# swapUniba/Deep_CBRS_Amar_Renaissance

Hardware: AMD Instinct MI355X
Metric: (user,item) pairs scored/sec, ML-1M basic-gnn 2-layer, 1/2/4/8 MI355X (higher is better)
Workload: dtype f32; 1 GPU; ml1m(s=64) user-item graph: N=590592 nodes, nnz(A_hat)=55909934, 12089292 test pairs; econfigs/basic-gnn.yaml grid1 BasicGCN d=8 L=2 concat, dense [24,24], clf [48,48]; one propagation + per-entity towers + all pairs (shuffled order) per step (hoisted); scale=64, parallelism=single GPU (step replayed from a hipGraph)

## Files before the change

deep_cbrs_amar_renaissance_amd/csrc/amar_chain.hip:

```cpp
#include "amar_common.h"
#include <stdlib.h>
#include <string.h>

namespace {

typedef float f32x4 __attribute__((ext_vector_type(4)));

constexpr int CHAIN_MAX_LAYERS = 8;
constexpr int CHAIN_MAX_SEG = 8;

struct ChainArgs {
    const float *A; int64_t lda; int Da; const int32_t *ids_a; int base_a;
    int n_seg; const float *seg[CHAIN_MAX_SEG]; int64_t seg_ld[CHAIN_MAX_SEG]; int seg_off[CHAIN_MAX_SEG + 1];
    const float *B; int64_t ldb; int Db; const int32_t *ids_b; int base_b;
    const float *wpack; int wpack_floats;
    int sum_inputs, in_act;
    int n_layers;
    int kt[CHAIN_MAX_LAYERS], nt[CHAIN_MAX_LAYERS], act[CHAIN_MAX_LAYERS];
    int w_off[CHAIN_MAX_LAYERS], b_off[CHAIN_MAX_LAYERS];
    int has_dot, dot_off, dot_bias_off, dot_act, dot_kt;
    int n_out;
    float *out; int64_t ldo; int64_t P;
    const int32_t *out_index;
};
// ... 132 lines not shown

__device__ __forceinline__ float relu_bits(float v) { return __int_as_float(max(__float_as_int(v), 0)); }

constexpr int chain_shape(int nl, int t0, int t1, int t2 = 0, int t3 = 0) { return nl | t0 << 3 | t1 << 6 | t2 << 9 | t3 << 12; }
constexpr int shape_nl(int s) { return s & 7; }
constexpr int shape_t(int s, int j) { return (s >> (3 * (j + 1))) & 7; }
constexpr int shape_maxt(int s) {
    int m = 0;
    for (int j = 0; j <= shape_nl(s); ++j) m = shape_t(s, j) > m ? shape_t(s, j) : m;
    return m;
}

template <int SHAPE, int PT, bool LASTLIN, bool SEG>
__global__ __launch_bounds__(256) void chain_rows_kernel(const ChainArgs a) {
    constexpr int NL = shape_nl(SHAPE), T0 = shape_t(SHAPE, 0), TN = shape_t(SHAPE, NL), MAXT = shape_maxt(SHAPE);
    extern __shared__ __attribute__((aligned(16))) float w_lds[];
    for (int i = threadIdx.x * 4; i < a.wpack_floats; i += blockDim.x * 4)
        *reinterpret_cast<float4 *>(&w_lds[i]) = *reinterpret_cast<const float4 *>(a.wpack + i);
    __syncthreads();

    const int lane = threadIdx.x & 63, g = lane >> 4, col = lane & 15;
    constexpr uint32_t rows_per_wave = 16 * PT;
    const uint32_t stride = gridDim.x * 4 * rows_per_wave;
    const uint32_t P = (uint32_t)a.P, last = P - 1;
    const uint32_t lda = (uint32_t)a.lda * 4u;
    const int f_last = 16 * (T0 - 1) + 4 * g;
    const bool tail_ok = f_last < a.Da;
    const char *Ag = reinterpret_cast<const char *>(a.A) + 16 * g;
    const int tail_off = tail_ok ? 64 * (T0 - 1) : -16 * g;
    const char *seg_base[SEG ? T0 : 1];
    uint32_t seg_ldb[SEG ? T0 : 1];
    if constexpr (SEG) {
#pragma unroll
        for (int t = 0; t < T0; ++t) {
            const int f = 16 * t + 4 * g;
            int sidx = 0;
            for (int j = 1; j < a.n_seg; ++j) sidx = (f < a.Da && f >= a.seg_off[j]) ? j : sidx;
            seg_base[t] = reinterpret_cast<const char *>(a.seg[sidx] + (f < a.Da ? f - a.seg_off[sidx] : 0));
            seg_ldb[t] = (uint32_t)a.seg_ld[sidx] * 4u;
        }
    }

    f32x4 xin[MAXT][PT];
    auto gather = [&](uint32_t b) {
#pragma unroll
        for (int pt = 0; pt < PT; ++pt) {
            const uint32_t p = min(b + 16 * pt + col, last);
            const uint32_t row = a.ids_a ? (uint32_t)(a.ids_a[p] - a.base_a) : p;
            const char *pa = Ag + (uint64_t)row * lda;
#pragma unroll
            for (int t = 0; t < T0; ++t) {
                if constexpr (SEG) xin[t][pt] = *reinterpret_cast<const f32x4 *>(seg_base[t] + (uint64_t)row * seg_ldb[t]);
                else xin[t][pt] = *reinterpret_cast<const f32x4 *>(pa + (t == T0 - 1 ? tail_off : 64 * t));
            }
        }
    };

    uint32_t base = (blockIdx.x * 4 + (threadIdx.x >> 6)) * rows_per_wave;
    if (base >= P) return;
    gather(base);
    for (; base < P; base += stride) {
        f32x4 x[MAXT][PT];
#pragma unroll
        for (int l = 0; l < NL; ++l) {
            const int KT = shape_t(SHAPE, l), NT = shape_t(SHAPE, l + 1);
            const float *wl = w_lds + a.w_off[l];
            const float *bl = w_lds + a.b_off[l];
            f32x4 y[MAXT][PT];
#pragma unroll
            for (int m = 0; m < MAXT; ++m) {
                if (m < NT) {
                    const f32x4 b4 = *reinterpret_cast<const f32x4 *>(bl + 16 * m + 4 * g);
#pragma unroll
                    for (int pt = 0; pt < PT; ++pt) y[m][pt] = b4;
#pragma unroll
                    for (int t = 0; t < MAXT; ++t) {
                        if (t < KT) {
                            const f32x4 w4 = *reinterpret_cast<const f32x4 *>(wl + ((m * KT + t) * 64 + lane) * 4);
#pragma unroll
                            for (int r = 0; r < 4; ++r)
#pragma unroll
                                for (int pt = 0; pt < PT; ++pt) {
                                    float xv = l == 0 ? xin[t][pt][r] : x[t][pt][r];
                                    if (l == 0 && t == T0 - 1) xv = tail_ok ? xv : 0.f;
                                    y[m][pt] = __builtin_amdgcn_mfma_f32_16x16x4f32(w4[r], xv, y[m][pt], 0, 0, 0);
                                }
                        }
                    }
                }
            }
            if (l == 0) gather(base + stride);
#pragma unroll
            for (int m = 0; m < MAXT; ++m)
#pragma unroll
                for (int pt = 0; pt < PT; ++pt)
                    if (m < NT) {
#pragma unroll
                        for (int r = 0; r < 4; ++r) x[m][pt][r] = (LASTLIN && l == NL - 1) ? y[m][pt][r] : relu_bits(y[m][pt][r]);
                    }
        }
#pragma unroll
        for (int pt = 0; pt < PT; ++pt) {
            const uint32_t p = base + 16 * pt + col;
            float *po = a.out + (int64_t)p * a.ldo + 4 * g;
#pragma unroll
            for (int m = 0; m < TN; ++m)
                if (p < P && 16 * m + 4 * g < a.n_out) *reinterpret_cast<f32x4 *>(po + 16 * m) = x[m][pt];
        }
    }
}


typedef uint32_t u32x4 __attribute__((ext_vector_type(4)));
typedef __bf16 bf16x8 __attribute__((ext_vector_type(8)));

struct Split3 { uint32_t h, m, l; };
typedef float f32x2 __attribute__((ext_vector_type(2)));
typedef uint32_t u32x2 __attribute__((ext_vector_type(2)));
__device__ __forceinline__ Split3 split_pair(float a, float b) {
    const f32x2 x = {a, b};
    const u32x2 xb = __builtin_bit_cast(u32x2, x);
    Split3 q;
    q.h = __builtin_amdgcn_perm(xb[1], xb[0], 0x07060302u);
    const f32x2 r1 = x - __builtin_bit_cast(f32x2, xb & 0xffff0000u);
    const u32x2 r1b = __builtin_bit_cast(u32x2, r1);
    q.m = __builtin_amdgcn_perm(r1b[1], r1b[0], 0x07060302u);
    const f32x2 r2 = r1 - __builtin_bit_cast(f32x2, r1b & 0xffff0000u);
    const u32x2 r2b = __builtin_bit_cast(u32x2, r2);
    q.l = __builtin_amdgcn_perm(r2b[1], r2b[0], 0x07060302u);
    return q;
}

struct Split3x4 { u32x4 h, m, l; };
__device__ __forceinline__ Split3x4 split_tiles(const f32x4 &t0, const f32x4 &t1) {
    const Split3 q0 = split_pair(t0[0], t0[1]), q1 = split_pair(t0[2], t0[3]), q2 = split_pair(t1[0], t1[1]), q3 = split_pair(t1[2], t1[3]);
    Split3x4 o;
    o.h[0] = q0.h; o.h[1] = q1.h; o.h[2] = q2.h; o.h[3] = q3.h;
    o.m[0] = q0.m; o.m[1] = q1.m; o.m[2] = q2.m; o.m[3] = q3.m;
    o.l[0] = q0.l; o.l[1] = q1.l; o.l[2] = q2.l; o.l[3] = q3.l;
    return o;
}
__device__ __forceinline__ f32x4 split_mfma(const u32x4 *w, const Split3x4 &x, f32x4 acc) {
    const bf16x8 wh = __builtin_bit_cast(bf16x8, w[0]), wm = __builtin_bit_cast(bf16x8, w[64]), wl = __builtin_bit_cast(bf16x8, w[128]);
    const bf16x8 xh = __builtin_bit_cast(bf16x8, x.h), xm = __builtin_bit_cast(bf16x8, x.m), xl = __builtin_bit_cast(bf16x8, x.l);
    acc = __builtin_amdgcn_mfma_f32_16x16x32_bf16(wl, xh, acc, 0, 0, 0);
    acc = __builtin_amdgcn_mfma_f32_16x16x32_bf16(wh, xl, acc, 0, 0, 0);
    acc = __builtin_amdgcn_mfma_f32_16x16x32_bf16(wm, xm, acc, 0, 0, 0);
    acc = __builtin_amdgcn_mfma_f32_16x16x32_bf16(wm, xh, acc, 0, 0, 0);
    acc = __builtin_amdgcn_mfma_f32_16x16x32_bf16(wh, xm, acc, 0, 0, 0);
    acc = __builtin_amdgcn_mfma_f32_16x16x32_bf16(wh, xh, acc, 0, 0, 0);
    return acc;
}

template <int MAXT, int PT, bool SCATTER, bool SPLIT>
__global__ __launch_bounds__(256) void chain_pipe_kernel(const ChainArgs a) {
    extern __shared__ __attribute__((aligned(16))) float w_lds[];
    for (int i = threadIdx.x * 4; i < a.wpack_floats; i += blockDim.x * 4)
        *reinterpret_cast<float4 *>(&w_lds[i]) = *reinterpret_cast<const float4 *>(a.wpack + i);
    __syncthreads();

    const int lane = threadIdx.x & 63, g = lane >> 4, col = lane & 15;
    constexpr int KS = (MAXT + 1) / 2;
    constexpr bool BIASK = SPLIT && (MAXT & 1);
    u32x4 *frag = reinterpret_cast<u32x4 *>(w_lds + ((a.wpack_floats + 3) & ~3));
    if (SPLIT) {
        for (int idx = threadIdx.x >> 6; idx < a.n_layers * MAXT * KS; idx += 4) {
            const int l = idx / (MAXT * KS), m = (idx % (MAXT * KS)) / KS, sk = idx % KS;
            const float *wl = w_lds + a.w_off[l];
            const f32x4 wa = *reinterpret_cast<const f32x4 *>(wl + ((m * MAXT + 2 * sk) * 64 + lane) * 4);
            f32x4 wb = {0.f, 0.f, 0.f, 0.f};
            if (2 * sk + 1 < MAXT) wb = *reinterpret_cast<const f32x4 *>(wl + ((m * MAXT + 2 * sk + 1) * 64 + lane) * 4);
            else if (BIASK && g == 0) wb[0] = w_lds[a.b_off[l] + 16 * m + col];
            u32x4 *dst = frag + idx * 3 * 64 + lane;
            const Split3 q0 = split_pair(wa[0], wa[1]), q1 = split_pair(wa[2], wa[3]), q2 = split_pair(wb[0], wb[1]), q3 = split_pair(wb[2], wb[3]);
            u32x4 h, mm, lo;
            h[0] = q0.h; h[1] = q1.h; h[2] = q2.h; h[3] = q3.h;
            mm[0] = q0.m; mm[1] = q1.m; mm[2] = q2.m; mm[3] = q3.m;
            lo[0] = q0.l; lo[1] = q1.l; lo[2] = q2.l; lo[3] = q3.l;
            dst[0] = h; dst[64] = mm; dst[128] = lo;
        }
        __syncthreads();
    }
    constexpr uint32_t pairs_per_wave = 16 * PT;
    const uint32_t wave0 = blockIdx.x * 4 + (threadIdx.x >> 6);
    const uint32_t stride = gridDim.x * 4 * pairs_per_wave;
    const uint32_t P = (uint32_t)a.P, last = P - 1;
    const char *Ag = reinterpret_cast<const char *>(a.A + 4 * g), *Bg = reinterpret_cast<const char *>(a.B + 4 * g);
    const uint32_t lda = (uint32_t)a.lda * 4u, ldb = (uint32_t)a.ldb * 4u;
    const char *ids_a = reinterpret_cast<const char *>(a.ids_a), *ids_b = reinterpret_cast<const char *>(a.ids_b);

    auto load_ids = [&](uint32_t b, int32_t (&ra)[PT], int32_t (&rb)[PT]) {
#pragma unroll
        for (int pt = 0; pt < PT; ++pt) {
            const uint32_t off = min(b + 16 * pt + col, last) << 2;
            ra[pt] = *reinterpret_cast<const int32_t *>(ids_a + off);
            rb[pt] = *reinterpret_cast<const int32_t *>(ids_b + off);
        }
    };
    auto issue = [&](const int32_t (&ra)[PT], const int32_t (&rb)[PT], f32x4 (&va)[MAXT][PT], f32x4 (&vb)[MAXT][PT]) {
#pragma unroll
        for (int pt = 0; pt < PT; ++pt) {
            const char *pa = Ag + (uint64_t)(uint32_t)(ra[pt] - a.base_a) * lda;
            const char *pb = Bg + (uint64_t)(uint32_t)(rb[pt] - a.base_b) * ldb;
#pragma unroll
            for (int t = 0; t < MAXT; ++t) {
                va[t][pt] = *reinterpret_cast<const f32x4 *>(pa + 64 * t);
                vb[t][pt] = *reinterpret_cast<const f32x4 *>(pb + 64 * t);
            }
        }
    };
#define AMAR_SPLIT_MFMA(W, X)                                                                                                   \
    _Pragma("unroll") for (int pt = 0; pt < PT; ++pt)                                                                           \
        y[m][pt] = __builtin_amdgcn_mfma_f32_16x16x32_bf16(W, __builtin_bit_cast(bf16x8, X[pt]), y[m][pt], 0, 0, 0)
    auto step = [&](uint32_t base, int32_t (&ra)[PT], int32_t (&rb)[PT], f32x4 (&va)[MAXT][PT], f32x4 (&vb)[MAXT][PT],
                    f32x4 (&na)[MAXT][PT], f32x4 (&nb)[MAXT][PT]) {
        int32_t out_row = 0;
        if (SCATTER) out_row = *reinterpret_cast<const int32_t *>(reinterpret_cast<const char *>(a.out_index) +
                                                                  (min(base + 16 * min(g, PT - 1) + col, last) << 2));
        f32x4 x[MAXT][PT];
#pragma unroll
        for (int t = 0; t < MAXT; ++t)
#pragma unroll
            for (int pt = 0; pt < PT; ++pt) {
                f32x4 v = va[t][pt] + vb[t][pt];
#pragma unroll
                for (int r = 0; r < 4; ++r) v[r] = relu_bits(v[r]);
                x[t][pt] = v;
            }
        issue(ra, rb, na, nb);
        load_ids(base + 2 * stride, ra, rb);
        for (int l = 0; SPLIT && l < a.n_layers; ++l) {
            u32x4 xq[3][KS][PT];
#pragma unroll
            for (int sk = 0; sk < KS; ++sk)
#pragma unroll
                for (int pt = 0; pt < PT; ++pt) {
#pragma unroll
                    for (int hf = 0; hf < 2; ++hf) {
                        const int t = 2 * sk + hf;
                        if (t < MAXT) {
                            const Split3 q0 = split_pair(x[t][pt][0], x[t][pt][1]), q1 = split_pair(x[t][pt][2], x[t][pt][3]);
                            xq[0][sk][pt][2 * hf] = q0.h; xq[1][sk][pt][2 * hf] = q0.m; xq[2][sk][pt][2 * hf] = q0.l;
                            xq[0][sk][pt][2 * hf + 1] = q1.h; xq[1][sk][pt][2 * hf + 1] = q1.m; xq[2][sk][pt][2 * hf + 1] = q1.l;
                        } else {
                            xq[0][sk][pt][2] = (BIASK && g == 0) ? 0x00003f80u : 0u;
                            xq[0][sk][pt][3] = 0u;
                            xq[1][sk][pt][2] = xq[1][sk][pt][3] = xq[2][sk][pt][2] = xq[2][sk][pt][3] = 0u;
                        }
                    }
                }
            const u32x4 *fl = frag + (size_t)l * MAXT * KS * 3 * 64 + lane;
            const float *bl = w_lds + a.b_off[l];
            f32x4 y[MAXT][PT];
#pragma unroll
            for (int m = 0; m < MAXT; ++m) {
                f32x4 b4 = {0.f, 0.f, 0.f, 0.f};
                if (!BIASK) b4 = *reinterpret_cast<const f32x4 *>(bl + 16 * m + 4 * g);
#pragma unroll
                for (int pt = 0; pt < PT; ++pt) y[m][pt] = b4;
#pragma unroll
                for (int sk = 0; sk < KS; ++sk) {
                    const bf16x8 wh = __builtin_bit_cast(bf16x8, fl[((m * KS + sk) * 3 + 0) * 64]);
                    const bf16x8 wm = __builtin_bit_cast(bf16x8, fl[((m * KS + sk) * 3 + 1) * 64]);
                    const bf16x8 wo = __builtin_bit_cast(bf16x8, fl[((m * KS + sk) * 3 + 2) * 64]);
                    AMAR_SPLIT_MFMA(wo, xq[0][sk]);
                    AMAR_SPLIT_MFMA(wh, xq[2][sk]);
                    AMAR_SPLIT_MFMA(wm, xq[1][sk]);
                    AMAR_SPLIT_MFMA(wm, xq[0][sk]);
                    AMAR_SPLIT_MFMA(wh, xq[1][sk]);
                    AMAR_SPLIT_MFMA(wh, xq[0][sk]);
                }
            }
#pragma unroll
            for (int m = 0; m < MAXT; ++m)
#pragma unroll
                for (int pt = 0; pt < PT; ++pt)
#pragma unroll
                    for (int r = 0; r < 4; ++r) x[m][pt][r] = relu_bits(y[m][pt][r]);
        }
        for (int l = 0; !SPLIT && l < a.n_layers; ++l) {
            const float *wl = w_lds + a.w_off[l] + lane * 4;
            const float *bl = w_lds + a.b_off[l];
            f32x4 y[MAXT][PT];
            f32x4 wnext = *reinterpret_cast<const f32x4 *>(wl);
#pragma unroll
            for (int m = 0; m < MAXT; ++m) {
                const f32x4 b4 = *reinterpret_cast<const f32x4 *>(bl + 16 * m + 4 * g);
#pragma unroll
                for (int pt = 0; pt < PT; ++pt) y[m][pt] = b4;
#pragma unroll
                for (int t = 0; t < MAXT; ++t) {
                    const f32x4 w4 = wnext;
                    if (m * MAXT + t + 1 < MAXT * MAXT) {
                        wnext = *reinterpret_cast<const f32x4 *>(wl + (m * MAXT + t + 1) * 256);
                        __builtin_amdgcn_sched_barrier(0);
                    }
#pragma unroll
                    for (int r = 0; r < 4; ++r)
#pragma unroll
                        for (int pt = 0; pt < PT; ++pt)
                            y[m][pt] = __builtin_amdgcn_mfma_f32_16x16x4f32(w4[r], x[t][pt][r], y[m][pt], 0, 0, 0);
                }
            }
#pragma unroll
            for (int m = 0; m < MAXT; ++m)
#pragma unroll
                for (int pt = 0; pt < PT; ++pt)
#pragma unroll
                    for (int r = 0; r < 4; ++r) x[m][pt][r] = relu_bits(y[m][pt][r]);
        }
        if (a.has_dot) {
            const float *wd = w_lds + a.dot_off;
            const float bd = w_lds[a.dot_bias_off];
            f32x4 w4[MAXT];
#pragma unroll
            for (int t = 0; t < MAXT; ++t) w4[t] = *reinterpret_cast<const f32x4 *>(wd + 16 * t + 4 * g);
            float s[PT];
#pragma unroll
            for (int pt = 0; pt < PT; ++pt) {
                float acc = 0.f;
#pragma unroll
                for (int t = 0; t < MAXT; ++t)
#pragma unroll
                    for (int r = 0; r < 4; ++r) acc = fmaf(x[t][pt][r], w4[t][r], acc);
                acc += __shfl_xor(acc, 16, 64);
                acc += __shfl_xor(acc, 32, 64);
                s[pt] = acc;
            }
            float z = s[0];
#pragma unroll
            for (int pt = 1; pt < PT; ++pt) z = g == pt ? s[pt] : z;
            z += bd;
            z = chain_act(z, a.dot_act);
            const uint32_t p = base + 16 * g + col;
            if (g < PT && p < P) a.out[(SCATTER ? (int64_t)out_row : (int64_t)p) * a.ldo] = z;
        } else {
#pragma unroll
            for (int pt = 0; pt < PT; ++pt) {
                const uint32_t p = base + 16 * pt + col;
#pragma unroll
                for (int m = 0; m < MAXT; ++m) {
                    const int f = 16 * m + 4 * g;
                    if (p < P && f < a.n_out) *reinterpret_cast<f32x4 *>(a.out + chain_out_row(a, p) * a.ldo + f) = x[m][pt];
                }
            }
        }
    };
#undef AMAR_SPLIT_MFMA

    uint32_t base = wave0 * pairs_per_wave;
    if (base >= P) return;
    f32x4 va[MAXT][PT], vb[MAXT][PT];
    int32_t ra[PT], rb[PT];
    load_ids(base, ra, rb);
    issue(ra, rb, va, vb);
    load_ids(base + stride, ra, rb);
    for (; base < P; base += stride) step(base, ra, rb, va, vb, va, vb);
}

struct DualArgs {
    const float *A[2]; int64_t lda[2]; const int32_t *ida[2]; int base_a[2];
    const float *B[2]; int64_t ldb[2]; const int32_t *idb[2]; int base_b[2];
    int D, tb, in_act;
    int n_branch; int bw_off[2][CHAIN_MAX_LAYERS], bb_off[2][CHAIN_MAX_LAYERS], b_act[CHAIN_MAX_LAYERS];
    int n_trunk, tt; int tw_off[CHAIN_MAX_LAYERS], tbias_off[CHAIN_MAX_LAYERS], t_act[CHAIN_MAX_LAYERS];
    int dot_off, dot_bias_off, dot_act;
    const float *wpack; int wpack_floats;
    float *out; int64_t ldo; int64_t P;
    const int32_t *out_index;
    int n_frag, tail_floats;
    int bw_frag[2][CHAIN_MAX_LAYERS], bb_tail[2][CHAIN_MAX_LAYERS], tw_frag[CHAIN_MAX_LAYERS], tb_tail[CHAIN_MAX_LAYERS], dot_tail, dot_bias_tail;
};

template <int PT>
__global__ __launch_bounds__(1024) void dual_chain_kernel(const DualArgs a) {
    constexpr int T = 4;
    extern __shared__ __attribute__((aligned(16))) float w_lds[];
    for (int i = threadIdx.x * 4; i < a.wpack_floats; i += blockDim.x * 4)
        *reinterpret_cast<float4 *>(&w_lds[i]) = *reinterpret_cast<const float4 *>(a.wpack + i);
    __syncthreads();
    const int lane = threadIdx.x & 63, g = lane >> 4, col = lane & 15;
    const int64_t pairs_per_wave = 16 * PT;
    const int wpb = blockDim.x >> 6;
    const int64_t wave0 = (int64_t)blockIdx.x * wpb + (threadIdx.x >> 6);
    const int64_t stride = (int64_t)gridDim.x * wpb * pairs_per_wave;
    const int TB = a.tb, TT = a.tt;

    for (int64_t base = wave0 * pairs_per_wave; base < a.P; base += stride) {
        f32x4 xb[2][T][PT];
#pragma unroll
        for (int br = 0; br < 2; ++br) {
#pragma unroll
            for (int pt = 0; pt < PT; ++pt) {
                const int64_t p = base + 16 * pt + col;
                const bool ok = p < a.P;
                const int64_t ra = ok ? (a.ida[br] ? (int64_t)a.ida[br][p] - a.base_a[br] : p) : 0;
                const int64_t rb = ok ? (a.idb[br] ? (int64_t)a.idb[br][p] - a.base_b[br] : p) : 0;
#pragma unroll
                for (int t = 0; t < T; ++t) {
                    const int f = 16 * t + 4 * g;
                    f32x4 v = {0.f, 0.f, 0.f, 0.f};
                    if (t < TB && ok && f < a.D) {
                        const f32x4 va = *reinterpret_cast<const f32x4 *>(a.A[br] + ra * a.lda[br] + f);
                        const f32x4 vb = *reinterpret_cast<const f32x4 *>(a.B[br] + rb * a.ldb[br] + f);
                        v = va + vb;
#pragma unroll
                        for (int r = 0; r < 4; ++r) v[r] = chain_act(v[r], a.in_act);
                    }
                    xb[br][t][pt] = v;
                }
            }
            for (int l = 0; l < a.n_branch; ++l) {
                const float *wl = w_lds + a.bw_off[br][l], *bl = w_lds + a.bb_off[br][l];
                f32x4 y[T][PT];
#pragma unroll
                for (int m = 0; m < T; ++m) {
                    if (m < TB) {
                        const f32x4 b4 = *reinterpret_cast<const f32x4 *>(bl + 16 * m + 4 * g);
#pragma unroll
                        for (int pt = 0; pt < PT; ++pt) y[m][pt] = b4;
#pragma unroll
                        for (int t = 0; t < T; ++t)
                            if (t < TB) {
                                const f32x4 w4 = *reinterpret_cast<const f32x4 *>(wl + ((m * TB + t) * 64 + lane) * 4);
#pragma unroll
                                for (int r = 0; r < 4; ++r)
#pragma unroll
                                    for (int pt = 0; pt < PT; ++pt)
                                        y[m][pt] = __builtin_amdgcn_mfma_f32_16x16x4f32(w4[r], xb[br][t][pt][r], y[m][pt], 0, 0, 0);
                            }
                    }
                }
#pragma unroll
                for (int m = 0; m < T; ++m)
#pragma unroll
                    for (int pt = 0; pt < PT; ++pt) {
                        f32x4 v = {0.f, 0.f, 0.f, 0.f};
                        if (m < TB) {
                            v = y[m][pt];
#pragma unroll
                            for (int r = 0; r < 4; ++r) v[r] = chain_act(v[r], a.b_act[l]);
                        }
                        xb[br][m][pt] = v;
                    }
            }
        }
        f32x4 x[T][PT];
        for (int l = 0; l < a.n_trunk; ++l) {
            const float *wl = w_lds + a.tw_off[l], *bl = w_lds + a.tbias_off[l];
            const int KT = l == 0 ? 2 * TB : TT;
            f32x4 y[T][PT];
#pragma unroll
            for (int m = 0; m < T; ++m) {
                if (m < TT) {
                    const f32x4 b4 = *reinterpret_cast<const f32x4 *>(bl + 16 * m + 4 * g);
#pragma unroll
                    for (int pt = 0; pt < PT; ++pt) y[m][pt] = b4;
#pragma unroll
                    for (int t = 0; t < 2 * T; ++t) {
                        const bool first = l == 0;
                        const int br = t >= T ? 1 : 0, tl = t >= T ? t - T : t;
                        const bool active = first ? (tl < TB) : (t < TT);
                        if (active) {
                            const int kt_idx = first ? (br * TB + tl) : t;
                            const f32x4 w4 = *reinterpret_cast<const f32x4 *>(wl + ((m * KT + kt_idx) * 64 + lane) * 4);
#pragma unroll
                            for (int r = 0; r < 4; ++r)
#pragma unroll
                                for (int pt = 0; pt < PT; ++pt) {
                                    const float bv = first ? xb[br][tl][pt][r] : (t < T ? x[t < T ? t : 0][pt][r] : 0.f);
                                    y[m][pt] = __builtin_amdgcn_mfma_f32_16x16x4f32(w4[r], bv, y[m][pt], 0, 0, 0);
                                }
                        }
                    }
                }
            }
#pragma unroll
            for (int m = 0; m < T; ++m)
#pragma unroll
                for (int pt = 0; pt < PT; ++pt) {
                    f32x4 v = {0.f, 0.f, 0.f, 0.f};
                    if (m < TT) {
                        v = y[m][pt];
#pragma unroll
                        for (int r = 0; r < 4; ++r) v[r] = chain_act(v[r], a.t_act[l]);
                    }
                    x[m][pt] = v;
                }
// ... 112 lines not shown
#pragma unroll
        for (int t = 0; t < T; ++t) {
            const f32x4 w4 = *reinterpret_cast<const f32x4 *>(wd + 16 * t + 4 * g);
#pragma unroll
            for (int r = 0; r < 4; ++r) sacc = fmaf(x[t][r], w4[r], sacc);
        }
        sacc += __shfl_xor(sacc, 16, 64);
        sacc += __shfl_xor(sacc, 32, 64);
        if (g == 0 && ok) a.out[(a.out_index ? (int64_t)a.out_index[p] : p) * a.ldo] = chain_act(sacc + w_lds[a.dot_bias_off], a.dot_act);
    }
}

template <int PT, int THREADS>
__global__ __launch_bounds__(THREADS) void dual_chain_split_kernel(const DualArgs a) {
    constexpr int T = 4, KS = 2;
    extern __shared__ __attribute__((aligned(16))) float w_lds[];
    u32x4 *frag = reinterpret_cast<u32x4 *>(w_lds);
    float *tail = w_lds + (size_t)a.n_frag * 3 * 64 * 4;
    const int lane = threadIdx.x & 63, g = lane >> 4, col = lane & 15;
    constexpr int wpb = THREADS / 64;
    const int wave = threadIdx.x >> 6;
    {
        auto build = [&](int w_off, int kt, int frag0) {
            const int ks = kt / 2;
            for (int f = wave; f < T * ks; f += wpb) {
                const int m = f / ks, sk = f % ks;
                const float *wl = a.wpack + w_off + ((size_t)(m * kt + 2 * sk) * 64 + lane) * 4;
                const Split3x4 q = split_tiles(*reinterpret_cast<const f32x4 *>(wl), *reinterpret_cast<const f32x4 *>(wl + 256));
                u32x4 *dst = frag + (size_t)(frag0 + f) * 3 * 64 + lane;
                dst[0] = q.h; dst[64] = q.m; dst[128] = q.l;
            }
        };
        for (int br = 0; br < 2; ++br)
            for (int l = 0; l < a.n_branch; ++l) build(a.bw_off[br][l], T, a.bw_frag[br][l]);
        for (int l = 0; l < a.n_trunk; ++l) build(a.tw_off[l], l == 0 ? 2 * T : T, a.tw_frag[l]);
        for (int i = threadIdx.x; i < 16 * T; i += THREADS) {
            for (int br = 0; br < 2; ++br)
                for (int l = 0; l < a.n_branch; ++l) tail[a.bb_tail[br][l] + i] = a.wpack[a.bb_off[br][l] + i];
            for (int l = 0; l < a.n_trunk; ++l) tail[a.tb_tail[l] + i] = a.wpack[a.tbias_off[l] + i];
            tail[a.dot_tail + i] = a.wpack[a.dot_off + i];
        }
        if (threadIdx.x == 0) tail[a.dot_bias_tail] = a.wpack[a.dot_bias_off];
    }
    __syncthreads();
    const int64_t wave0 = (int64_t)blockIdx.x * wpb + wave;
    const int64_t stride = (int64_t)gridDim.x * wpb * 16 * PT;

    auto layer_step = [&](const u32x4 *w, const Split3x4 (&x)[PT], f32x4 (&y)[PT]) {
        const bf16x8 wh = __builtin_bit_cast(bf16x8, w[0]), wm = __builtin_bit_cast(bf16x8, w[64]), wl = __builtin_bit_cast(bf16x8, w[128]);
#define AMAR_DUAL_MFMA(W, PART)                                                                                                  \
    _Pragma("unroll") for (int pt = 0; pt < PT; ++pt)                                                                            \
        y[pt] = __builtin_amdgcn_mfma_f32_16x16x32_bf16(W, __builtin_bit_cast(bf16x8, x[pt].PART), y[pt], 0, 0, 0)
        AMAR_DUAL_MFMA(wl, h); AMAR_DUAL_MFMA(wh, l); AMAR_DUAL_MFMA(wm, m); AMAR_DUAL_MFMA(wm, h); AMAR_DUAL_MFMA(wh, m); AMAR_DUAL_MFMA(wh, h);
#undef AMAR_DUAL_MFMA
    };

    for (int64_t base = wave0 * 16 * PT; base < a.P; base += stride) {
        Split3x4 xq[2][KS][PT];
#pragma unroll
        for (int br = 0; br < 2; ++br) {
#pragma unroll
            for (int pt = 0; pt < PT; ++pt) {
                const int64_t p = base + 16 * pt + col;
                const bool ok = p < a.P;
                const uint32_t ra = ok ? (uint32_t)(a.ida[br][p] - a.base_a[br]) : 0u;
                const uint32_t rb = ok ? (uint32_t)(a.idb[br][p] - a.base_b[br]) : 0u;
                const float *pa = a.A[br] + (uint64_t)ra * (uint32_t)a.lda[br] + 4 * g;
                const float *pb = a.B[br] + (uint64_t)rb * (uint32_t)a.ldb[br] + 4 * g;
                f32x4 xb[T];
#pragma unroll
                for (int t = 0; t < T; ++t) {
                    f32x4 v = *reinterpret_cast<const f32x4 *>(pa + 16 * t) + *reinterpret_cast<const f32x4 *>(pb + 16 * t);
#pragma unroll
                    for (int r = 0; r < 4; ++r) v[r] = relu_bits(v[r]);
                    xb[t] = v;
                }
#pragma unroll
                for (int sk = 0; sk < KS; ++sk) xq[br][sk][pt] = split_tiles(xb[2 * sk], xb[2 * sk + 1]);
            }
            for (int l = 0; l < a.n_branch; ++l) {
                const u32x4 *fl = frag + (size_t)a.bw_frag[br][l] * 3 * 64 + lane;
                const float *bl = tail + a.bb_tail[br][l];
                f32x4 y[T][PT];
#pragma unroll
                for (int m = 0; m < T; ++m) {
                    const f32x4 b4 = *reinterpret_cast<const f32x4 *>(bl + 16 * m + 4 * g);
#pragma unroll
                    for (int pt = 0; pt < PT; ++pt) y[m][pt] = b4;
#pragma unroll
                    for (int sk = 0; sk < KS; ++sk) layer_step(fl + (m * KS + sk) * 3 * 64, xq[br][sk], y[m]);
                }
#pragma unroll
                for (int pt = 0; pt < PT; ++pt) {
#pragma unroll
                    for (int m = 0; m < T; ++m)
#pragma unroll
                        for (int r = 0; r < 4; ++r) y[m][pt][r] = relu_bits(y[m][pt][r]);
#pragma unroll
                    for (int sk = 0; sk < KS; ++sk) xq[br][sk][pt] = split_tiles(y[2 * sk][pt], y[2 * sk + 1][pt]);
                }
            }
        }
        f32x4 x[T][PT];
        Split3x4 xt[KS][PT];
        for (int l = 0; l < a.n_trunk; ++l) {
            const u32x4 *fl = frag + (size_t)a.tw_frag[l] * 3 * 64 + lane;
            const float *bl = tail + a.tb_tail[l];
            f32x4 y[T][PT];
#pragma unroll
            for (int m = 0; m < T; ++m) {
                const f32x4 b4 = *reinterpret_cast<const f32x4 *>(bl + 16 * m + 4 * g);
#pragma unroll
                for (int pt = 0; pt < PT; ++pt) y[m][pt] = b4;
                if (l == 0) {
#pragma unroll
                    for (int sk = 0; sk < 2 * KS; ++sk) layer_step(fl + (m * 2 * KS + sk) * 3 * 64, xq[sk / KS][sk % KS], y[m]);
                } else {
#pragma unroll
                    for (int sk = 0; sk < KS; ++sk) layer_step(fl + (m * KS + sk) * 3 * 64, xt[sk], y[m]);
                }
            }
#pragma unroll
            for (int pt = 0; pt < PT; ++pt) {
#pragma unroll
                for (int m = 0; m < T; ++m)
#pragma unroll
                    for (int r = 0; r < 4; ++r) x[m][pt][r] = relu_bits(y[m][pt][r]);
                if (l + 1 < a.n_trunk) {
#pragma unroll
                    for (int sk = 0; sk < KS; ++sk) xt[sk][pt] = split_tiles(x[2 * sk][pt], x[2 * sk + 1][pt]);
                }
            }
        }
        const float *wd = tail + a.dot_tail;
        f32x4 w4[T];
#pragma unroll
        for (int t = 0; t < T; ++t) w4[t] = *reinterpret_cast<const f32x4 *>(wd + 16 * t + 4 * g);
#pragma unroll
        for (int pt = 0; pt < PT; ++pt) {
            float sacc = 0.f;
#pragma unroll
            for (int t = 0; t < T; ++t)
#pragma unroll
                for (int r = 0; r < 4; ++r) sacc = fmaf(x[t][pt][r], w4[t][r], sacc);
            sacc += __shfl_xor(sacc, 16, 64);
            sacc += __shfl_xor(sacc, 32, 64);
            const int64_t p = base + 16 * pt + col;
            if (g == 0 && p < a.P) a.out[(a.out_index ? (int64_t)a.out_index[p] : p) * a.ldo] = chain_act(sacc + tail[a.dot_bias_tail], a.dot_act);
        }
    }
}

inline int tiles16(int n) { return (n + 15) / 16; }

}

extern "C" {

int64_t amar_chain_pack_floats(const int32_t *dims, int32_t n_layers) {
    if (!dims || n_layers < 1 || n_layers > CHAIN_MAX_LAYERS) return AMAR_EINVAL;
    int64_t total = 0;
    for (int l = 0; l < n_layers; ++l) {
        const int K = dims[l], N = dims[l + 1];
        if (K < 1 || N < 1) return AMAR_EINVAL;
        if (l == n_layers - 1 && N == 1 && n_layers > 1) total += 16 * tiles16(K) + 4;
        else total += (int64_t)tiles16(N) * tiles16(K) * 256 + 16 * tiles16(N);
    }
    return total;
}

int amar_chain_pack_f32(const float *const *kernels, const float *const *biases, const int32_t *dims,
                        int32_t n_layers, float *out) {
    if (!kernels || !biases || !out) return AMAR_EINVAL;
    const int64_t total = amar_chain_pack_floats(dims, n_layers);
    if (total < 0) return (int)total;
    int64_t off = 0;
    for (int l = 0; l < n_layers; ++l) {
        const int K = dims[l], N = dims[l + 1], KT = tiles16(K), NT = tiles16(N);
        const float *W = kernels[l], *b = biases[l];
        if (l == n_layers - 1 && N == 1 && n_layers > 1) {
            for (int k = 0; k < 16 * KT; ++k) out[off + k] = k < K ? W[k] : 0.f;
            off += 16 * KT;
            out[off] = b[0]; out[off + 1] = out[off + 2] = out[off + 3] = 0.f;
            off += 4;
        } else {
            for (int m = 0; m < NT; ++m)
                for (int t = 0; t < KT; ++t)
                    for (int lane = 0; lane < 64; ++lane)
                        for (int r = 0; r < 4; ++r) {
                            const int k = 16 * t + 4 * (lane >> 4) + r, n = 16 * m + (lane & 15);
                            out[off++] = (k < K && n < N) ? W[(int64_t)k * N + n] : 0.f;
                        }
            for (int n = 0; n < 16 * NT; ++n) out[off++] = n < N ? b[n] : 0.f;
        }
    }
    return off == total ? AMAR_OK : AMAR_EINVAL;
}

int amar_chain_f32(const float *A, int64_t lda, int32_t Da, const int32_t *ids_a, int32_t base_a,
                   const float *B, int64_t ldb, int32_t Db, const int32_t *ids_b, int32_t base_b,
                   int32_t sum_inputs, int32_t in_act,
                   const float *wpack, const int32_t *dims, const int32_t *acts, int32_t n_layers,
                   float *out, int64_t ldo, int64_t P, amar_stream_t stream) {
    return amar_chain_indexed_f32(A, lda, Da, ids_a, base_a, B, ldb, Db, ids_b, base_b, sum_inputs, in_act, wpack, dims, acts, n_layers,
                                  out, ldo, nullptr, P, stream);
}

static int chain_run(const float *A, int64_t lda, int32_t Da, const int32_t *ids_a, int32_t base_a,
                     const float *B, int64_t ldb, int32_t Db, const int32_t *ids_b, int32_t base_b,
                     int32_t sum_inputs, int32_t in_act,
                     const float *wpack, const int32_t *dims, const int32_t *acts, int32_t n_layers,
                     float *out, int64_t ldo, const int32_t *out_index, int64_t P, amar_stream_t stream,
                     int32_t n_seg, const float *const *seg, const int64_t *seg_ld, const int32_t *seg_width);

int amar_chain_indexed_f32(const float *A, int64_t lda, int32_t Da, const int32_t *ids_a, int32_t base_a,
                           const float *B, int64_t ldb, int32_t Db, const int32_t *ids_b, int32_t base_b,
                           int32_t sum_inputs, int32_t in_act,
                           const float *wpack, const int32_t *dims, const int32_t *acts, int32_t n_layers,
                           float *out, int64_t ldo, const int32_t *out_index, int64_t P, amar_stream_t stream) {
    return chain_run(A, lda, Da, ids_a, base_a, B, ldb, Db, ids_b, base_b, sum_inputs, in_act, wpack, dims, acts, n_layers, out, ldo, out_index, P,
                     stream, 0, nullptr, nullptr, nullptr);
}

int amar_chain_segments_f32(const float *const *seg, const int64_t *seg_ld, const int32_t *seg_width, int32_t n_seg,
                            const int32_t *ids, int32_t base,
                            const float *wpack, const int32_t *dims, const int32_t *acts, int32_t n_layers,
                            float *out, int64_t ldo, int64_t P, amar_stream_t stream) {
    if (!seg || !seg_ld || !seg_width || n_seg < 1 || n_seg > CHAIN_MAX_SEG) return AMAR_EINVAL;
    int64_t da = 0;
    for (int j = 0; j < n_seg; ++j) {
        if (!seg[j] || seg_width[j] < 4 || (seg_width[j] & 3) || seg_ld[j] < seg_width[j] || (seg_ld[j] & 3) || !amar_aligned16(seg[j]) ||
            seg_ld[j] >= (1ll << 30))
            return AMAR_EINVAL;
        da += seg_width[j];
    }
    if (da > 128) return AMAR_EUNSUPPORTED;
    return chain_run(seg[0], seg_ld[0], (int32_t)da, ids, base, nullptr, 0, 0, nullptr, 0, 0, AMAR_ACT_NONE, wpack, dims, acts, n_layers, out, ldo,
                     nullptr, P, stream, n_seg, seg, seg_ld, seg_width);
}

static int chain_run(const float *A, int64_t lda, int32_t Da, const int32_t *ids_a, int32_t base_a,
                     const float *B, int64_t ldb, int32_t Db, const int32_t *ids_b, int32_t base_b,
                     int32_t sum_inputs, int32_t in_act,
                     const float *wpack, const int32_t *dims, const int32_t *acts, int32_t n_layers,
                     float *out, int64_t ldo, const int32_t *out_index, int64_t P, amar_stream_t stream,
                     int32_t n_seg, const float *const *seg, const int64_t *seg_ld, const int32_t *seg_width) {
    if (P < 0 || !A || !wpack || !dims || !acts || !out || Da < 4 || Db < 0) return AMAR_EINVAL;
    if (sum_inputs && (Db != Da || !B)) return AMAR_EINVAL;
    if (in_act != AMAR_ACT_NONE && in_act != AMAR_ACT_RELU && in_act != AMAR_ACT_SIGMOID) return AMAR_EINVAL;
    if ((Da & 3) || (Db & 3) || (lda & 3) || (n_seg == 0 && lda < Da) || !amar_aligned16(A) || !amar_aligned16(wpack)) return AMAR_EINVAL;
    if (Db && (!B || (ldb & 3) || ldb < Db || !amar_aligned16(B))) return AMAR_EINVAL;
    if (n_layers < 1 || n_layers > CHAIN_MAX_LAYERS || dims[0] != (sum_inputs ? Da : Da + Db)) return AMAR_EINVAL;
    ChainArgs a{};
    a.A = A; a.lda = lda; a.Da = Da; a.ids_a = ids_a; a.base_a = base_a;
    a.B = B; a.ldb = ldb; a.Db = Db; a.ids_b = ids_b; a.base_b = base_b;
    a.wpack = wpack; a.out = out; a.ldo = ldo; a.P = P; a.sum_inputs = sum_inputs ? 1 : 0; a.in_act = in_act;
    a.out_index = out_index;
    a.n_seg = n_seg;
    for (int j = 0; j < n_seg; ++j) {
        a.seg[j] = seg[j]; a.seg_ld[j] = seg_ld[j];
        a.seg_off[j + 1] = a.seg_off[j] + seg_width[j];
    }
    int maxw = 0, off = 0;
    for (int l = 0; l < n_layers; ++l) {
        const int K = dims[l], N = dims[l + 1], act = acts[l];
        if (K < 1 || N < 1 || (act != AMAR_ACT_NONE && act != AMAR_ACT_RELU && act != AMAR_ACT_SIGMOID)) return AMAR_EINVAL;
        maxw = K > maxw ? K : maxw;
        if (l == n_layers - 1 && N == 1 && n_layers > 1) {
            a.has_dot = 1; a.dot_off = off; a.dot_kt = tiles16(K); a.dot_act = act;
            off += 16 * tiles16(K);
            a.dot_bias_off = off;
            off += 4;
        } else {
            maxw = N > maxw ? N : maxw;
            a.kt[a.n_layers] = tiles16(K); a.nt[a.n_layers] = tiles16(N); a.act[a.n_layers] = act;
            a.w_off[a.n_layers] = off;
            off += tiles16(N) * tiles16(K) * 256;
            a.b_off[a.n_layers] = off;
            off += 16 * tiles16(N);
            a.n_layers++;
            a.n_out = N;
        }
    }
    a.wpack_floats = off;
    if (a.n_layers < 1) return AMAR_EINVAL;
    if (!a.has_dot && ((ldo & 3) || ldo < a.n_out || (a.n_out & 3) || !amar_aligned16(out))) return AMAR_EINVAL;
    if (a.has_dot && ldo < 1) return AMAR_EINVAL;
    if (maxw > 128 || (size_t)off * sizeof(float) > 150 * 1024) return AMAR_EUNSUPPORTED;
    if (P == 0) return AMAR_OK;
    const size_t lds_bytes = (size_t)off * sizeof(float);
    hipStream_t st = static_cast<hipStream_t>(stream);
    const int maxt = maxw <= 48 ? 3 : (maxw <= 64 ? 4 : 8);
    bool full = (dims[0] + 15) / 16 == maxt && (!a.has_dot || a.dot_kt == maxt);
    for (int l = 0; l < a.n_layers; ++l) full = full && a.kt[l] == maxt && a.nt[l] == maxt;
    bool relu = !a.sum_inputs || a.in_act == AMAR_ACT_RELU, relu_but_last = relu && !a.has_dot;
    for (int l = 0; l < a.n_layers; ++l) {
        relu = relu && a.act[l] == AMAR_ACT_RELU;
        relu_but_last = relu_but_last && a.act[l] == (l == a.n_layers - 1 ? AMAR_ACT_NONE : AMAR_ACT_RELU);
    }
    const int am = relu ? 1 : (relu_but_last ? 2 : 0);
#define AMAR_CHAIN_LAUNCH(MT)                                                                                           \
    do {                                                                                                                \
        int64_t blocks = (P + 4 * 16 * 2 - 1) / (4 * 16 * 2);                                                           \
        if (blocks > 4096) blocks = 4096;                                                                               \
        auto kern = full ? (am == 1 ? chain_kernel<MT, 2, true, 1> : am == 2 ? chain_kernel<MT, 2, true, 2>             \
                                                                             : chain_kernel<MT, 2, true, 0>)            \
                         : (am == 1 ? chain_kernel<MT, 2, false, 1> : am == 2 ? chain_kernel<MT, 2, false, 2>           \
                                                                              : chain_kernel<MT, 2, false, 0>);         \
        if (lds_bytes > 64 * 1024 &&                                                                                    \
            hipFuncSetAttribute(reinterpret_cast<const void *>(kern), hipFuncAttributeMaxDynamicSharedMemorySize,       \
                                (int)lds_bytes) != hipSuccess)                                                          \
            return AMAR_ELAUNCH;                                                                                        \
        hipLaunchKernelGGL(kern, dim3((unsigned)blocks), dim3(256), lds_bytes, st, a);                                  \
    } while (0)
    const bool a_dot_ok = !a.has_dot || a.dot_kt == maxt;
    const bool small_tables = lda < (1ll << 30) && ldb < (1ll << 30) && P < (1ll << 30) - (4ll << 20);
    if (relu && a.sum_inputs && a.in_act == AMAR_ACT_RELU && full && a_dot_ok && a.ids_a && a.ids_b && a.Da == 16 * maxt &&
        a.Db == a.Da && maxt <= 4 && lds_bytes <= 64 * 1024 && small_tables) {
        int64_t blocks = (P + 4 * 16 * 2 - 1) / (4 * 16 * 2);
        if (blocks > 1536) blocks = 1536;
        const dim3 grid((unsigned)blocks), block(256);
        if (a.out_index && !a.has_dot) return AMAR_EUNSUPPORTED;
        static const bool f32_only = getenv("AMAR_PAIR_MFMA") && !strcmp(getenv("AMAR_PAIR_MFMA"), "f32");
        const size_t split_bytes = (((size_t)off + 3) & ~(size_t)3) * sizeof(float) + (size_t)a.n_layers * maxt * ((maxt + 1) / 2) * 3 * 1024;
        const bool split = !f32_only && split_bytes <= 64 * 1024;
        const size_t lds = split ? split_bytes : lds_bytes;
#define AMAR_PIPE_LAUNCH(MT, SC)                                                                                          \
        do {                                                                                                              \
            if (split) hipLaunchKernelGGL((chain_pipe_kernel<MT, 2, SC, true>), grid, block, lds, st, a);                 \
            else hipLaunchKernelGGL((chain_pipe_kernel<MT, 2, SC, false>), grid, block, lds, st, a);                      \
        } while (0)
        if (a.out_index) {
            if (maxt == 3) AMAR_PIPE_LAUNCH(3, true); else AMAR_PIPE_LAUNCH(4, true);
        } else {
            if (maxt == 3) AMAR_PIPE_LAUNCH(3, false); else AMAR_PIPE_LAUNCH(4, false);
        }
#undef AMAR_PIPE_LAUNCH
        return amar_check_launch();
    }
    if ((am == 1 || am == 2) && !a.sum_inputs && a.Db == 0 && !a.has_dot && !a.out_index && a.n_layers <= 3 &&
        maxt <= 4 && lds_bytes <= 64 * 1024 && lda < (1ll << 30) && P < (1ll << 30) - (4ll << 20)) {
        const int shape = chain_shape(a.n_layers, a.kt[0], a.nt[0], a.n_layers > 1 ? a.nt[1] : 0, a.n_layers > 2 ? a.nt[2] : 0);
        int64_t blocks = (P + 4 * 16 * 2 - 1) / (4 * 16 * 2);
        if (blocks > 1024) blocks = 1024;
        const dim3 grid((unsigned)blocks), block(256);
        bool done = true;
#define AMAR_ROWS_CASE(NLL, A0, A1, A2, A3)                                                                                      \
        case chain_shape(NLL, A0, A1, A2, A3):                                                                                   \
            if (n_seg > 0) {                                                                                                     \
                if (am == 2) hipLaunchKernelGGL((chain_rows_kernel<chain_shape(NLL, A0, A1, A2, A3), 2, true, true>), grid, block, lds_bytes, st, a);   \
                else hipLaunchKernelGGL((chain_rows_kernel<chain_shape(NLL, A0, A1, A2, A3), 2, false, true>), grid, block, lds_bytes, st, a);          \
            } else if (am == 2) hipLaunchKernelGGL((chain_rows_kernel<chain_shape(NLL, A0, A1, A2, A3), 2, true, false>), grid, block, lds_bytes, st, a);   \
            else hipLaunchKernelGGL((chain_rows_kernel<chain_shape(NLL, A0, A1, A2, A3), 2, false, false>), grid, block, lds_bytes, st, a);          \
            break
        switch (shape) {
        AMAR_ROWS_CASE(3, 2, 2, 2, 3);
        AMAR_ROWS_CASE(3, 3, 3, 3, 4);
        AMAR_ROWS_CASE(2, 2, 2, 2, 0);
        AMAR_ROWS_CASE(3, 1, 2, 2, 3);
        AMAR_ROWS_CASE(3, 1, 3, 3, 4);
        AMAR_ROWS_CASE(2, 3, 3, 3, 0);
        default: done = false;
        }
#undef AMAR_ROWS_CASE
        if (done) return amar_check_launch();
    }
    if (n_seg > 0) return AMAR_EUNSUPPORTED;
    if (maxt == 3) AMAR_CHAIN_LAUNCH(3); else if (maxt == 4) AMAR_CHAIN_LAUNCH(4); else AMAR_CHAIN_LAUNCH(8);
#undef AMAR_CHAIN_LAUNCH
    return amar_check_launch();
}

int amar_dual_chain_f32(const float *const *A, const int64_t *lda, const int32_t *const *ida, const int32_t *base_a,
                        const float *const *B, const int64_t *ldb, const int32_t *const *idb, const int32_t *base_b,
                        int32_t D, int32_t in_act, int32_t n_branch, const int32_t *branch_acts,
                        const int32_t *trunk_dims, const int32_t *trunk_acts, int32_t n_trunk,
                        const float *wpack, float *out, int64_t ldo, int64_t P, amar_stream_t stream) {
    return amar_dual_chain_indexed_f32(A, lda, ida, base_a, B, ldb, idb, base_b, D, in_act, n_branch, branch_acts, trunk_dims, trunk_acts,
                                       n_trunk, wpack, out, ldo, nullptr, P, stream);
}

int amar_dual_chain_indexed_f32(const float *const *A, const int64_t *lda, const int32_t *const *ida, const int32_t *base_a,
                                const float *const *B, const int64_t *ldb, const int32_t *const *idb, const int32_t *base_b,
                                int32_t D, int32_t in_act, int32_t n_branch, const int32_t *branch_acts,
                                const int32_t *trunk_dims, const int32_t *trunk_acts, int32_t n_trunk,
                                const float *wpack, float *out, int64_t ldo, const int32_t *out_index, int64_t P, amar_stream_t stream) {
    if (P < 0 || !A || !B || !lda || !ldb || !ida || !idb || !base_a || !base_b || !wpack || !out || !trunk_dims || !trunk_acts)
        return AMAR_EINVAL;
    if (D < 4 || (D & 3) || n_branch < 0 || n_branch > CHAIN_MAX_LAYERS || (n_branch && !branch_acts)) return AMAR_EINVAL;
    if (n_trunk < 2 || n_trunk > CHAIN_MAX_LAYERS || trunk_dims[0] != 2 * D || trunk_dims[n_trunk] != 1 || ldo < 1) return AMAR_EINVAL;
    if (D > 64) return AMAR_EUNSUPPORTED;
    DualArgs a{};
    for (int b = 0; b < 2; ++b) {
        if (!A[b] || !B[b] || lda[b] < D || ldb[b] < D || (lda[b] & 3) || (ldb[b] & 3) || !amar_aligned16(A[b]) || !amar_aligned16(B[b]))
            return AMAR_EINVAL;
        a.A[b] = A[b]; a.lda[b] = lda[b]; a.ida[b] = ida[b]; a.base_a[b] = base_a[b];
        a.B[b] = B[b]; a.ldb[b] = ldb[b]; a.idb[b] = idb[b]; a.base_b[b] = base_b[b];
    }
    a.D = D; a.tb = tiles16(D); a.in_act = in_act; a.n_branch = n_branch;
    int off = 0;
    for (int b = 0; b < 2; ++b)
        for (int l = 0; l < n_branch; ++l) {
            a.bw_off[b][l] = off; off += a.tb * a.tb * 256;
            a.bb_off[b][l] = off; off += 16 * a.tb;
            a.b_act[l] = branch_acts[l];
        }
    const int W = trunk_dims[1];
    if (W < 4 || (W & 3) || W > 64) return AMAR_EUNSUPPORTED;
    a.tt = tiles16(W); a.n_trunk = n_trunk - 1;
    for (int l = 0; l < n_trunk - 1; ++l) {
        if (trunk_dims[l + 1] != W) return AMAR_EUNSUPPORTED;
        const int KT = l == 0 ? 2 * a.tb : a.tt;
        if (l == 0 && (D & 15)) return AMAR_EUNSUPPORTED;
        a.tw_off[l] = off; off += a.tt * KT * 256;
        a.tbias_off[l] = off; off += 16 * a.tt;
        a.t_act[l] = trunk_acts[l];
    }
    a.dot_off = off; off += 16 * a.tt;
    a.dot_bias_off = off; off += 4;
    a.dot_act = trunk_acts[n_trunk - 1];
    a.wpack = wpack; a.wpack_floats = off; a.out = out; a.ldo = ldo; a.P = P; a.out_index = out_index;
    if ((size_t)off * sizeof(float) > 150 * 1024) return AMAR_EUNSUPPORTED;
    if (P == 0) return AMAR_OK;
    const size_t lds_bytes = (size_t)off * sizeof(float);
    constexpr int PT = 1;
    constexpr int THREADS = 1024;
    int64_t blocks = (P + (THREADS / 64) * 16 * PT - 1) / ((THREADS / 64) * 16 * PT);
    if (blocks > 1024) blocks = 1024;
    bool full = D == 64 && W == 64 && in_act == AMAR_ACT_RELU && n_branch >= 1 && ida[0] && ida[1] && idb[0] && idb[1];
    for (int b = 0; b < 2; ++b) full = full && lda[b] < (1ll << 32) && ldb[b] < (1ll << 32);
    for (int l = 0; l < n_branch; ++l) full = full && branch_acts[l] == AMAR_ACT_RELU;
    for (int l = 0; l < n_trunk - 1; ++l) full = full && trunk_acts[l] == AMAR_ACT_RELU;
    static const bool f32_only = getenv("AMAR_PAIR_MFMA") && !strcmp(getenv("AMAR_PAIR_MFMA"), "f32");
    if (full && !f32_only && n_branch >= 1) {
        int nf = 0, tl = 0;
        for (int b = 0; b < 2; ++b)
            for (int l = 0; l < n_branch; ++l) { a.bw_frag[b][l] = nf; nf += 4 * 2; a.bb_tail[b][l] = tl; tl += 64; }
        for (int l = 0; l < a.n_trunk; ++l) { a.tw_frag[l] = nf; nf += 4 * (l == 0 ? 4 : 2); a.tb_tail[l] = tl; tl += 64; }
        a.dot_tail = tl; tl += 64; a.dot_bias_tail = tl; tl += 4;
        a.n_frag = nf; a.tail_floats = tl;
        const size_t bytes = (size_t)nf * 3 * 1024 + (size_t)tl * sizeof(float);
        if (bytes <= 160 * 1024) {
            static bool lds_ok[AMAR_MAX_DEVICES];
            if (bytes > 64 * 1024)
                if (const int rc = amar_allow_lds(reinterpret_cast<const void *>(dual_chain_split_kernel<1, 768>), 160 * 1024, lds_ok)) return rc;
            int64_t blocks3 = (P + 12 * 16 - 1) / (12 * 16);
            if (blocks3 > 1024) blocks3 = 1024;
            hipLaunchKernelGGL((dual_chain_split_kernel<1, 768>), dim3((unsigned)blocks3), dim3(768), bytes, static_cast<hipStream_t>(stream), a);
            return amar_check_launch();
        }
    }
    auto kern = full ? dual_chain_full_kernel : dual_chain_kernel<PT>;
    if (lds_bytes > 64 * 1024 &&
        hipFuncSetAttribute(reinterpret_cast<const void *>(kern), hipFuncAttributeMaxDynamicSharedMemorySize, (int)lds_bytes) != hipSuccess)
        return AMAR_ELAUNCH;
    hipLaunchKernelGGL(kern, dim3((unsigned)blocks), dim3(THREADS), lds_bytes, static_cast<hipStream_t>(stream), a);
    return amar_check_launch();
}

}
```

Before: 11.84 billion pairs/s.

## Specialize pair pipeline kernel on layer count, prefetch weight fragments, size grid by occupancy

Adds a compile-time layer count so the split-bf16 pair kernel can fully unroll its layer loop and carry a dot head with a simplified output store. The kernel also gets waves-per-EU hints and a sched_barrier. Weight fragments are software-prefetched one step ahead from LDS so each load overlaps the MFMAs of the previous step. The grid cap moves from a fixed 1536 blocks to a value derived from occupancy queries (two waves of resident blocks, capped at 8192). The aim is to cut LDS load latency and loop overhead and fill the GPU better, at the cost of more template instantiations and possible register pressure from the occupancy hints.

```diff
diff --git a/deep_cbrs_amar_renaissance_amd/csrc/amar_chain.hip b/deep_cbrs_amar_renaissance_amd/csrc/amar_chain.hip
--- a/deep_cbrs_amar_renaissance_amd/csrc/amar_chain.hip
+++ b/deep_cbrs_amar_renaissance_amd/csrc/amar_chain.hip
@@ -308,19 +308,23 @@
     return acc;
 }
 
-template <int MAXT, int PT, bool SCATTER, bool SPLIT>
-__global__ __launch_bounds__(256) void chain_pipe_kernel(const ChainArgs a) {
+
+template <int MAXT, int PT, bool SCATTER, bool SPLIT, int NL>
+__global__ __launch_bounds__(256) __attribute__((amdgpu_waves_per_eu((SPLIT && NL == 1 && MAXT == 3) ? 3 : (SPLIT && NL ? 2 : 1))))
+void chain_pipe_kernel(const ChainArgs a) {
     extern __shared__ __attribute__((aligned(16))) float w_lds[];
     for (int i = threadIdx.x * 4; i < a.wpack_floats; i += blockDim.x * 4)
         *reinterpret_cast<float4 *>(&w_lds[i]) = *reinterpret_cast<const float4 *>(a.wpack + i);
     __syncthreads();
+    constexpr bool HEAD = NL > 0;
+    const int n_layers = HEAD ? NL : a.n_layers;
 
     const int lane = threadIdx.x & 63, g = lane >> 4, col = lane & 15;
     constexpr int KS = (MAXT + 1) / 2;
     constexpr bool BIASK = SPLIT && (MAXT & 1);
     u32x4 *frag = reinterpret_cast<u32x4 *>(w_lds + ((a.wpack_floats + 3) & ~3));
     if (SPLIT) {
-        for (int idx = threadIdx.x >> 6; idx < a.n_layers * MAXT * KS; idx += 4) {
+        for (int idx = threadIdx.x >> 6; idx < n_layers * MAXT * KS; idx += 4) {
             const int l = idx / (MAXT * KS), m = (idx % (MAXT * KS)) / KS, sk = idx % KS;
             const float *wl = w_lds + a.w_off[l];
             const f32x4 wa = *reinterpret_cast<const f32x4 *>(wl + ((m * MAXT + 2 * sk) * 64 + lane) * 4);
@@ -385,7 +389,8 @@
             }
         issue(ra, rb, na, nb);
         load_ids(base + 2 * stride, ra, rb);
-        for (int l = 0; SPLIT && l < a.n_layers; ++l) {
+#pragma unroll
+        for (int l = 0; SPLIT && l < n_layers; ++l) {
             u32x4 xq[3][KS][PT];
 #pragma unroll
             for (int sk = 0; sk < KS; ++sk)
@@ -408,6 +413,9 @@
             const u32x4 *fl = frag + (size_t)l * MAXT * KS * 3 * 64 + lane;
             const float *bl = w_lds + a.b_off[l];
             f32x4 y[MAXT][PT];
+            u32x4 wnext[3];
+#pragma unroll
+            for (int part = 0; part < 3; ++part) wnext[part] = fl[part * 64];
 #pragma unroll
             for (int m = 0; m < MAXT; ++m) {
                 f32x4 b4 = {0.f, 0.f, 0.f, 0.f};
@@ -416,9 +424,13 @@
                 for (int pt = 0; pt < PT; ++pt) y[m][pt] = b4;
 #pragma unroll
                 for (int sk = 0; sk < KS; ++sk) {
-                    const bf16x8 wh = __builtin_bit_cast(bf16x8, fl[((m * KS + sk) * 3 + 0) * 64]);
-                    const bf16x8 wm = __builtin_bit_cast(bf16x8, fl[((m * KS + sk) * 3 + 1) * 64]);
-                    const bf16x8 wo = __builtin_bit_cast(bf16x8, fl[((m * KS + sk) * 3 + 2) * 64]);
+                    const bf16x8 wh = __builtin_bit_cast(bf16x8, wnext[0]), wm = __builtin_bit_cast(bf16x8, wnext[1]);
+                    const bf16x8 wo = __builtin_bit_cast(bf16x8, wnext[2]);
+                    if (m * KS + sk + 1 < MAXT * KS) {
+#pragma unroll
+                        for (int part = 0; part < 3; ++part) wnext[part] = fl[((m * KS + sk + 1) * 3 + part) * 64];
+                    }
+                    if (HEAD) __builtin_amdgcn_sched_barrier(0x211);
                     AMAR_SPLIT_MFMA(wo, xq[0][sk]);
                     AMAR_SPLIT_MFMA(wh, xq[2][sk]);
                     AMAR_SPLIT_MFMA(wm, xq[1][sk]);
@@ -434,7 +446,7 @@
 #pragma unroll
                     for (int r = 0; r < 4; ++r) x[m][pt][r] = relu_bits(y[m][pt][r]);
         }
-        for (int l = 0; !SPLIT && l < a.n_layers; ++l) {
+        for (int l = 0; !SPLIT && l < n_layers; ++l) {
             const float *wl = w_lds + a.w_off[l] + lane * 4;
             const float *bl = w_lds + a.b_off[l];
             f32x4 y[MAXT][PT];
@@ -465,7 +477,7 @@
 #pragma unroll
                     for (int r = 0; r < 4; ++r) x[m][pt][r] = relu_bits(y[m][pt][r]);
         }
-        if (a.has_dot) {
+        if (HEAD || a.has_dot) {
             const float *wd = w_lds + a.dot_off;
             const float bd = w_lds[a.dot_bias_off];
             f32x4 w4[MAXT];
@@ -489,7 +501,9 @@
             z += bd;
             z = chain_act(z, a.dot_act);
             const uint32_t p = base + 16 * g + col;
-            if (g < PT && p < P) a.out[(SCATTER ? (int64_t)out_row : (int64_t)p) * a.ldo] = z;
+            if (HEAD) {
+                if (g < PT && p < P) a.out[SCATTER ? (uint32_t)out_row : p] = z;
+            } else if (g < PT && p < P) a.out[(SCATTER ? (int64_t)out_row : (int64_t)p) * a.ldo] = z;
         } else {
 #pragma unroll
             for (int pt = 0; pt < PT; ++pt) {
@@ -908,6 +922,24 @@
 }
 
 inline int tiles16(int n) { return (n + 15) / 16; }
+
+template <void (*KERN)(const ChainArgs)>
+void pipe_launch(int64_t P, size_t lds, hipStream_t st, const ChainArgs &a) {
+    thread_local size_t seen_lds = ~(size_t)0;
+    thread_local int64_t cap = 1536;
+    if (seen_lds != lds) {
+        int dev = 0, cus = 0, resident = 0;
+        cap = 1536;
+        if (hipGetDevice(&dev) == hipSuccess && hipDeviceGetAttribute(&cus, hipDeviceAttributeMultiprocessorCount, dev) == hipSuccess &&
+            hipOccupancyMaxActiveBlocksPerMultiprocessor(&resident, KERN, 256, lds) == hipSuccess && cus > 0 && resident > 0)
+            cap = ((int64_t)cus * resident * 2 + 7) & ~(int64_t)7;
+        if (cap > 8192) cap = 8192;
+        seen_lds = lds;
+    }
+    int64_t blocks = (P + 127) / 128;
+    if (blocks > cap) blocks = cap;
+    hipLaunchKernelGGL(KERN, dim3((unsigned)blocks), dim3(256), lds, st, a);
+}
 
 }
 
@@ -1073,18 +1105,18 @@
     const bool small_tables = lda < (1ll << 30) && ldb < (1ll << 30) && P < (1ll << 30) - (4ll << 20);
     if (relu && a.sum_inputs && a.in_act == AMAR_ACT_RELU && full && a_dot_ok && a.ids_a && a.ids_b && a.Da == 16 * maxt &&
         a.Db == a.Da && maxt <= 4 && lds_bytes <= 64 * 1024 && small_tables) {
-        int64_t blocks = (P + 4 * 16 * 2 - 1) / (4 * 16 * 2);
-        if (blocks > 1536) blocks = 1536;
-        const dim3 grid((unsigned)blocks), block(256);
         if (a.out_index && !a.has_dot) return AMAR_EUNSUPPORTED;
         static const bool f32_only = getenv("AMAR_PAIR_MFMA") && !strcmp(getenv("AMAR_PAIR_MFMA"), "f32");
         const size_t split_bytes = (((size_t)off + 3) & ~(size_t)3) * sizeof(float) + (size_t)a.n_layers * maxt * ((maxt + 1) / 2) * 3 * 1024;
         const bool split = !f32_only && split_bytes <= 64 * 1024;
         const size_t lds = split ? split_bytes : lds_bytes;
+        const int nl = (a.has_dot && ldo == 1 && a.n_layers <= 2) ? a.n_layers : 0;
 #define AMAR_PIPE_LAUNCH(MT, SC)                                                                                          \
         do {                                                                                                              \
-            if (split) hipLaunchKernelGGL((chain_pipe_kernel<MT, 2, SC, true>), grid, block, lds, st, a);                 \
-            else hipLaunchKernelGGL((chain_pipe_kernel<MT, 2, SC, false>), grid, block, lds, st, a);                      \
+            if (split && nl == 1) pipe_launch<chain_pipe_kernel<MT, 2, SC, true, 1>>(P, lds, st, a);                      \
+            else if (split && nl == 2) pipe_launch<chain_pipe_kernel<MT, 2, SC, true, 2>>(P, lds, st, a);                 \
+            else if (split) pipe_launch<chain_pipe_kernel<MT, 2, SC, true, 0>>(P, lds, st, a);                            \
+            else pipe_launch<chain_pipe_kernel<MT, 2, SC, false, 0>>(P, lds_bytes, st, a);                                \
         } while (0)
         if (a.out_index) {
             if (maxt == 3) AMAR_PIPE_LAUNCH(3, true); else AMAR_PIPE_LAUNCH(4, true);
```

After: 11.73 billion pairs/s. No clear change (-1.0%).
